# olegroshka/vae-channel-dynamics

Hardware: AMD Instinct MI355X
Metric: images/sec SDXL-VAE train step @256x256 (tracking on) (higher is better)
Workload: dtype f32

## Files before the change

### vae-channel-dynamics_amd/csrc/wgrad3_wino.hip

```cpp
#include "common.h"
#ifndef VAE_ABLATE
#define VAE_ABLATE 0
#endif
#include <algorithm>
#include <type_traits>

namespace {

constexpr int GCI = 32, GCO = 128, GNT = 512;
constexpr int XS = 20;
constexpr int SXF = 4 * GCI * XS;
constexpr int SYF = 2 * GCO * XS;
constexpr int GSTAGE = SXF + SYF;

template <int XF>
__global__ __launch_bounds__(GNT, 1) void wgrad3_wino_kernel(vae_wgrad_args p, int strips, int64_t nunits) {
  __shared__ __attribute__((aligned(16))) float smem[2 * GSTAGE];

  const int tid = threadIdx.x, lane = tid & 63, wave = tid >> 6;
  const int lr = lane & 31, lh = lane >> 5;
  const vae_conv_geom g = p.g;
  const int tilesN = p.N / GCI, ntile = tilesN * (p.M / GCO);
  int tile, split;
  {
    const int L = blockIdx.x, ns = p.nsplit;
    if (ns % 8 == 0) {
      const int j = L >> 3;
      tile = j % ntile;
      split = (j / ntile) * 8 + (L & 7);
    } else if ((ns == 2 || ns == 4) && ntile % (8 / ns) == 0) {
      split = (L & 7) % ns;
      tile = (L >> 3) * (8 / ns) + (L & 7) / ns;
    } else {
      tile = L % ntile;
      split = L / ntile;
    }
  }
  const int tm = tile / tilesN, tn = tile % tilesN;
  const int m0 = tm * GCO, n0 = tn * GCI;
  const int64_t per = (nunits + p.nsplit - 1) / p.nsplit;
  const int64_t ubeg = split * per, uend = min(nunits, ubeg + per);
  const int nu = (int)max((int64_t)0, uend - ubeg);
  const int upi = (g.Ho / 2) * strips;
  const bool do_bias = (p.bias_partial != nullptr) && tn == 0;

  const int xx = tid & 15, xq = (tid >> 4) & 7, xr = tid >> 7;
  const bool xe_role = tid < 128 && (tid & 8) == 0;
  const int ex = 16 + (tid & 1), er = (tid >> 1) & 3;
  const int yq = tid >> 4;
  const auto rsX = VAE_BUF_RSRC(p.X, (size_t)g.B * g.Hs * g.Ws * g.Cs * 4u);
  const auto rsY = VAE_BUF_RSRC(p.dY, (size_t)g.B * g.Ho * g.Wo * p.ldy * 4u);
  struct Stg {
    f32x4 rx, rxe, ry[2];
    int b;
    bool xin, xein;
  };
  const f32x4 z4 = {0.f, 0.f, 0.f, 0.f};
  Stg s0{z4, z4, {z4, z4}, -1, false, false}, s1 = s0;
  f32x4 bsum = z4;
  f32x4 rsc = {1.f, 1.f, 1.f, 1.f}, rsh = z4;
  int sc_b = -1;
  int ub = (int)(ubeg / upi), uty = (int)((ubeg - (int64_t)ub * upi) / strips), ustrip = (int)((ubeg - (int64_t)ub * upi) % strips);
  const unsigned thrX = ((xr * g.Ws + xx) * g.Cs + n0 + 4 * xq) * 4u, thrE = ((er * g.Ws + ex) * g.Cs + n0 + 4 * xq) * 4u;
  const unsigned thrY = (xx * p.ldy + m0 + 4 * yq) * 4u, rowY = (unsigned)g.Wo * p.ldy * 4u;
  const int tfX = (xr == 0 ? 1 : 0) | (xr == 3 ? 2 : 0) | (xx == 0 ? 4 : 0) | 16;
  const int tfE = xe_role ? ((er == 0 ? 1 : 0) | (er == 3 ? 2 : 0) | (ex == 17 ? 8 : 0) | 16) : 31;
  auto load_unit = [&](int k, Stg& r) {
    const bool ok = k < nu;
    const int b = ub, ty = uty, x0 = ustrip * 16;
    if (++ustrip == strips) {
      ustrip = 0;
      if (++uty == g.Ho / 2) {
        uty = 0;
        ++ub;
      }
    }
    r.b = ok ? b : -1;
    const int uf = (ty == 0 ? 1 : 0) | (2 * ty + 2 >= g.Hs ? 2 : 0) | (x0 == 0 ? 4 : 0) | (x0 + 16 >= g.Ws ? 8 : 0) | (ok ? 0 : 16);
    const unsigned baseX = (unsigned)((b * g.Hs + 2 * ty - 1) * g.Ws + x0 - 1) * (unsigned)g.Cs * 4u;
    const unsigned baseY = (unsigned)((b * g.Ho + 2 * ty) * g.Wo + x0) * (unsigned)p.ldy * 4u;
    r.xin = (tfX & uf) == 0;
    r.rx = VAE_BUF_LOAD4(rsX, r.xin ? baseX + thrX : BUF_OOB);
    r.xein = (tfE & uf) == 0;
    r.rxe = VAE_BUF_LOAD4(rsX, r.xein ? baseX + thrE : BUF_OOB);
#pragma unroll
    for (int a = 0; a < 2; ++a) r.ry[a] = VAE_BUF_LOAD4(rsY, ok ? baseY + a * rowY + thrY : BUF_OOB);
  };
  auto xform = [&](f32x4 v, bool in) {
    if (XF != VAE_XF_NONE) {
#pragma unroll
      for (int e = 0; e < 4; ++e) {
        float u = v[e] * rsc[e] + rsh[e];
        if (XF == VAE_XF_AFFINE_SILU) u = silu_f(u);
        v[e] = in ? u : 0.f;
      }
    }
    return v;
  };
  auto store_unit = [&](float* st, const Stg& r) {
    float* sx = st;
    float* sy = st + SXF;
    if (XF != VAE_XF_NONE && r.b >= 0 && r.b != sc_b) {
      sc_b = r.b;
      rsc = *reinterpret_cast<const f32x4*>(p.scale + (int64_t)sc_b * g.Cs + n0 + 4 * xq);
      rsh = *reinterpret_cast<const f32x4*>(p.shift + (int64_t)sc_b * g.Cs + n0 + 4 * xq);
    }
    const f32x4 v = xform(r.rx, r.xin);
#pragma unroll
    for (int e = 0; e < 4; ++e) sx[(xr * GCI + 4 * xq + e) * XS + xx] = v[e];
    if (xe_role) {
      const f32x4 ve = xform(r.rxe, r.xein);
#pragma unroll
      for (int e = 0; e < 4; ++e) sx[(er * GCI + 4 * xq + e) * XS + ex] = ve[e];
    }
#pragma unroll
    for (int a = 0; a < 2; ++a) {
#pragma unroll
      for (int e = 0; e < 4; ++e) sy[(a * GCO + 4 * yq + e) * XS + xx] = r.ry[a][e];
      if (do_bias) bsum += r.ry[a];
    }
  };

  const int wi = wave >> 1, jh = wave & 1;
  const int vr1 = wi == 0 ? 0 : (wi == 2 ? 2 : 1), vr2 = wi == 0 ? 2 : (wi == 1 ? 2 : (wi == 2 ? 1 : 3));
  const int voff1 = (vr1 * GCI + lr) * XS + 8 * lh, voff2 = (vr2 * GCI + lr) * XS + 8 * lh;
  const int dr1 = wi == 3 ? 1 : 0;

  f32x16 acc[2][4];
#pragma unroll
  for (int pi = 0; pi < 2; ++pi)
#pragma unroll
    for (int nb = 0; nb < 4; ++nb)
#pragma unroll
      for (int e = 0; e < 16; ++e) acc[pi][nb][e] = 0.f;

  load_unit(0, s0);
  store_unit(smem, s0);
  load_unit(1, s1);
  __syncthreads();

  auto run = [&](auto WI, auto JH) {
    constexpr int wic = decltype(WI)::value, jhc = decltype(JH)::value;
    constexpr bool two = wic == 1 || wic == 2;
    constexpr bool vplus = wic == 1;
    auto step = [&](int k, const Stg& cur, Stg& nxt) {
      const float* cx = smem + (k & 1) * GSTAGE;
      const float* cy = cx + SXF;
      float* nst = smem + ((k + 1) & 1) * GSTAGE;
      f32x4 rd[2][2];
      auto read_d = [&](int nb, f32x4 (&d)[2][2]) {
        const int doff = (dr1 * GCO + nb * 32 + lr) * XS + 8 * lh;
#pragma unroll
        for (int c = 0; c < 2; ++c) {
          d[0][c] = *reinterpret_cast<const f32x4*>(&cy[doff + 4 * c]);
          if (two) d[1][c] = *reinterpret_cast<const f32x4*>(&cy[doff + GCO * XS + 4 * c]);
        }
      };
      auto build_b = [&](const f32x4 (&d)[2][2], f32x4 (&b4)[2]) {
        float rc[8];
#pragma unroll
        for (int c = 0; c < 2; ++c)
#pragma unroll
          for (int e = 0; e < 4; ++e) rc[4 * c + e] = !two ? d[0][c][e] : (vplus ? d[0][c][e] + d[1][c][e] : d[0][c][e] - d[1][c][e]);
#pragma unroll
        for (int e = 0; e < 4; ++e) {
          if (jhc == 0) {
            b4[0][e] = rc[2 * e];
            b4[1][e] = rc[2 * e] + rc[2 * e + 1];
          } else {
            b4[0][e] = rc[2 * e] - rc[2 * e + 1];
            b4[1][e] = rc[2 * e + 1];
          }
        }
      };
      f32x4 a4[2], bb[2][2];
      {
        f32x4 u1[3], u2[3];
#pragma unroll
        for (int c = 0; c < 3; ++c) {
          u1[c] = *reinterpret_cast<const f32x4*>(&cx[voff1 + 4 * c]);
          u2[c] = *reinterpret_cast<const f32x4*>(&cx[voff2 + 4 * c]);
        }
        float rc[12];
#pragma unroll
        for (int c = 0; c < 3; ++c)
#pragma unroll
          for (int e = 0; e < 4; ++e) rc[4 * c + e] = vplus ? u1[c][e] + u2[c][e] : u1[c][e] - u2[c][e];
        __builtin_amdgcn_sched_barrier(0);
        read_d(0, rd);
#pragma unroll
        for (int e = 0; e < 4; ++e) {
          if (jhc == 0) {
            a4[0][e] = rc[2 * e] - rc[2 * e + 2];
            a4[1][e] = rc[2 * e + 1] + rc[2 * e + 2];
          } else {
            a4[0][e] = rc[2 * e + 2] - rc[2 * e + 1];
            a4[1][e] = rc[2 * e + 1] - rc[2 * e + 3];
          }
        }
        build_b(rd, bb[0]);
        read_d(1, rd);
      }
      if (!(VAE_ABLATE & 2) && wave < 4) store_unit(nst, cur);
#pragma unroll
      for (int nb = 0; nb < 4; ++nb) {
        __builtin_amdgcn_sched_barrier(0);
        if (nb == 1) {
          if (!(VAE_ABLATE & 1)) load_unit(k + 2, nxt);
          __builtin_amdgcn_sched_barrier(0);
        }
        if (nb == 3 && wave >= 4) {
          if (!(VAE_ABLATE & 2)) store_unit(nst, cur);
          __builtin_amdgcn_sched_barrier(0);
        }
        if (nb < 3) build_b(rd, bb[(nb + 1) & 1]);
        if (nb < 2) read_d(nb + 2, rd);
#pragma unroll
        for (int pi = 0; pi < 2; ++pi)
#pragma unroll
          for (int e = 0; e < 4; ++e) acc[pi][nb] = __builtin_amdgcn_mfma_f32_32x32x2f32(a4[pi][e], bb[nb & 1][pi][e], acc[pi][nb], 0, 0, 0);
#pragma unroll
        for (int i = 0; i < 4; ++i) {
          __builtin_amdgcn_sched_group_barrier(0x008, 1, 0);
          __builtin_amdgcn_sched_group_barrier(0x002, 3, 0);
        }
        __builtin_amdgcn_sched_group_barrier(0x100, 4, 0);
        __builtin_amdgcn_sched_group_barrier(0x008, 4, 0);
        __builtin_amdgcn_sched_barrier(0);
      }
      if (!(VAE_ABLATE & 16)) __syncthreads();
    };
    int k = 0;
    for (; k + 1 < nu; k += 2) {
      step(k, s1, s0);
      step(k + 1, s0, s1);
    }
    if (k < nu) step(k, s1, s0);
  };
  {
    using J0 = std::integral_constant<int, 0>;
    using J1 = std::integral_constant<int, 1>;
    switch (wave) {
      case 0: run(std::integral_constant<int, 0>{}, J0{}); break;
      case 1: run(std::integral_constant<int, 0>{}, J1{}); break;
      case 2: run(std::integral_constant<int, 1>{}, J0{}); break;
      case 3: run(std::integral_constant<int, 1>{}, J1{}); break;
      case 4: run(std::integral_constant<int, 2>{}, J0{}); break;
      case 5: run(std::integral_constant<int, 2>{}, J1{}); break;
      case 6: run(std::integral_constant<int, 3>{}, J0{}); break;
      default: run(std::integral_constant<int, 3>{}, J1{}); break;
    }
  }

  float* __restrict__ O = p.partial + (int64_t)split * 16 * p.N * p.M;
#pragma unroll
  for (int pi = 0; pi < 2; ++pi) {
    const int pos = wi * 4 + 2 * jh + pi;
#pragma unroll
    for (int nb = 0; nb < 4; ++nb)
#pragma unroll
      for (int e = 0; e < 16; ++e) {
        const int ci = n0 + (e & 3) + 8 * (e >> 2) + 4 * lh;
        O[((int64_t)pos * p.N + ci) * p.M + m0 + nb * 32 + lr] = acc[pi][nb][e];
      }
  }
  if (do_bias) {
#pragma unroll
    for (int e = 0; e < 4; ++e) {
      float s = bsum[e];
#pragma unroll
      for (int o = 1; o < 16; o <<= 1) s += __shfl_xor(s, o, 64);
      if (xx == 0) p.bias_partial[(int64_t)split * p.M + m0 + 4 * yq + e] = s;
    }
  }
}

}

bool wgrad3_wino_eligible(const vae_wgrad_args& a) {
  const vae_conv_geom& g = a.g;
  if (a.prec != VAE_PREC_F32 || a.X16 != nullptr || a.dY16 != nullptr || a.dY == nullptr || a.batch != 1 || a.alpha != 1.0f) return false;
  if (g.taps != 9 || g.stride != 1 || g.pad_t != 1 || g.pad_l != 1 || g.mode != VAE_MODE_FWD) return false;
  if (a.tapmask != 0 || a.y_step > 1 || g.Ho != g.Hs || g.Wo != g.Ws) return false;
  if (g.Ho % 2 != 0 || g.Wo % 16 != 0 || a.N % GCI != 0 || a.M % GCO != 0 || g.Cs % 4 != 0 || a.ldy % 4 != 0) return false;
  if (!aligned16(a.X) || !aligned16(a.dY)) return false;
  if ((size_t)g.B * g.Hs * g.Ws * g.Cs * 4u >= BUF_MAX || (size_t)g.B * g.Ho * g.Wo * a.ldy * 4u >= BUF_MAX) return false;
  return true;
}

int64_t wgrad3_wino_units(const vae_conv_geom& g) { return (int64_t)g.B * (g.Ho / 2) * (g.Wo / 16); }

int launch_wgrad3_wino(const vae_wgrad_args& a, hipStream_t st) {
  const vae_conv_geom& g = a.g;
  const int64_t nunits = wgrad3_wino_units(g);
  dim3 grid((unsigned)((a.M / GCO) * (a.N / GCI) * a.nsplit), 1, 1);
  const int strips = g.Wo / 16;
  if (a.xf == VAE_XF_NONE) hipLaunchKernelGGL(wgrad3_wino_kernel<VAE_XF_NONE>, grid, dim3(GNT), 0, st, a, strips, nunits);
  else if (a.xf == VAE_XF_AFFINE) hipLaunchKernelGGL(wgrad3_wino_kernel<VAE_XF_AFFINE>, grid, dim3(GNT), 0, st, a, strips, nunits);
  else hipLaunchKernelGGL(wgrad3_wino_kernel<VAE_XF_AFFINE_SILU>, grid, dim3(GNT), 0, st, a, strips, nunits);
  return 0;
}
```

Baseline: 104.4.

## Defer last channel-block MFMAs of waves 4-7 past the barrier into next step

For waves 4-7, which store the next stage late in the step, the MFMAs for the last one or two channel blocks (default two) are held back and issued at the start of the following step, after the __syncthreads. The goal is to shorten those waves' critical path before the barrier so all waves reach the sync sooner, with the deferred matrix work overlapping the next step's LDS reads. The a4/bb operands move out of the step so they persist across steps, and a final flush runs after the loop. Optional timing instrumentation is added but compiled only when VAE_WGRAD_TIMING is defined.

Result: faster. 106.7 (median of 6 runs) (+2.1%).

```diff
diff --git a/vae-channel-dynamics_amd/csrc/wgrad3_wino.hip b/vae-channel-dynamics_amd/csrc/wgrad3_wino.hip
--- a/vae-channel-dynamics_amd/csrc/wgrad3_wino.hip
+++ b/vae-channel-dynamics_amd/csrc/wgrad3_wino.hip
@@ -1,6 +1,9 @@
 #include "common.h"
 #ifndef VAE_ABLATE
 #define VAE_ABLATE 0
+#endif
+#ifndef VAE_WGRAD_DEFER
+#define VAE_WGRAD_DEFER 2
 #endif
 #include <algorithm>
 #include <type_traits>
@@ -43,6 +46,18 @@
   const int nu = (int)max((int64_t)0, uend - ubeg);
   const int upi = (g.Ho / 2) * strips;
   const bool do_bias = (p.bias_partial != nullptr) && tn == 0;
+#ifdef VAE_WGRAD_TIMING
+  constexpr int TS0 = 2, TSN = 8;
+  const bool tw = (tid & 255) == 0 && blockIdx.x < 8 && p.out != nullptr;
+  unsigned long long* const tout = reinterpret_cast<unsigned long long*>(p.out) + (blockIdx.x * 2 + (tid >> 8)) * (4 + TSN * 5);
+  unsigned long long tst[5];
+  const unsigned long long te0 = __builtin_amdgcn_s_memtime(), tr0 = __builtin_amdgcn_s_memrealtime();
+#define GSTAMP(i) do { __builtin_amdgcn_sched_barrier(0); tst[i] = __builtin_amdgcn_s_memtime(); __builtin_amdgcn_sched_barrier(0); } while (0)
+#define GSTAMPS_OUT(k) do { if (tw && (k) >= TS0 && (k) < TS0 + TSN) { _Pragma("unroll") for (int i_ = 0; i_ < 5; ++i_) tout[4 + ((k) - TS0) * 5 + i_] = tst[i_]; } } while (0)
+#else
+#define GSTAMP(i) do { } while (0)
+#define GSTAMPS_OUT(k) do { } while (0)
+#endif
 
   const int xx = tid & 15, xq = (tid >> 4) & 7, xr = tid >> 7;
   const bool xe_role = tid < 128 && (tid & 8) == 0;
@@ -143,10 +158,32 @@
     constexpr int wic = decltype(WI)::value, jhc = decltype(JH)::value;
     constexpr bool two = wic == 1 || wic == 2;
     constexpr bool vplus = wic == 1;
+    constexpr int ndef = wic >= 2 ? VAE_WGRAD_DEFER : 0;
+    static_assert(ndef >= 0 && ndef <= 2, "bb holds the operands of two channel blocks");
+    f32x4 a4[2], bb[2][2];
+    if (ndef > 0) {
+      a4[0] = a4[1] = z4;
+      bb[0][0] = bb[0][1] = bb[1][0] = bb[1][1] = z4;
+    }
+    auto held_back = [&]() {
+#pragma unroll
+      for (int e = 0; e < 4; ++e)
+#pragma unroll
+        for (int nb = 4 - ndef; nb < 4; ++nb)
+#pragma unroll
+          for (int pi = 0; pi < 2; ++pi) acc[pi][nb] = __builtin_amdgcn_mfma_f32_32x32x2f32(a4[pi][e], bb[nb & 1][pi][e], acc[pi][nb], 0, 0, 0);
+    };
     auto step = [&](int k, const Stg& cur, Stg& nxt) {
       const float* cx = smem + (k & 1) * GSTAGE;
       const float* cy = cx + SXF;
       float* nst = smem + ((k + 1) & 1) * GSTAGE;
+      GSTAMP(0);
+      if (ndef > 0) {
+        __builtin_amdgcn_sched_barrier(0);
+        held_back();
+        __builtin_amdgcn_sched_barrier(0);
+      }
+      GSTAMP(1);
       f32x4 rd[2][2];
       auto read_d = [&](int nb, f32x4 (&d)[2][2]) {
         const int doff = (dr1 * GCO + nb * 32 + lr) * XS + 8 * lh;
@@ -173,7 +210,6 @@
           }
         }
       };
-      f32x4 a4[2], bb[2][2];
       {
         f32x4 u1[3], u2[3];
 #pragma unroll
@@ -202,6 +238,7 @@
         read_d(1, rd);
       }
       if (!(VAE_ABLATE & 2) && wave < 4) store_unit(nst, cur);
+      GSTAMP(2);
 #pragma unroll
       for (int nb = 0; nb < 4; ++nb) {
         __builtin_amdgcn_sched_barrier(0);
@@ -215,19 +252,24 @@
         }
         if (nb < 3) build_b(rd, bb[(nb + 1) & 1]);
         if (nb < 2) read_d(nb + 2, rd);
-#pragma unroll
-        for (int pi = 0; pi < 2; ++pi)
-#pragma unroll
-          for (int e = 0; e < 4; ++e) acc[pi][nb] = __builtin_amdgcn_mfma_f32_32x32x2f32(a4[pi][e], bb[nb & 1][pi][e], acc[pi][nb], 0, 0, 0);
-#pragma unroll
-        for (int i = 0; i < 4; ++i) {
-          __builtin_amdgcn_sched_group_barrier(0x008, 1, 0);
-          __builtin_amdgcn_sched_group_barrier(0x002, 3, 0);
-        }
-        __builtin_amdgcn_sched_group_barrier(0x100, 4, 0);
-        __builtin_amdgcn_sched_group_barrier(0x008, 4, 0);
-        __builtin_amdgcn_sched_barrier(0);
-      }
+        if (nb < 4 - ndef) {
+#pragma unroll
+          for (int pi = 0; pi < 2; ++pi)
+#pragma unroll
+            for (int e = 0; e < 4; ++e) acc[pi][nb] = __builtin_amdgcn_mfma_f32_32x32x2f32(a4[pi][e], bb[nb & 1][pi][e], acc[pi][nb], 0, 0, 0);
+#pragma unroll
+          for (int i = 0; i < 4; ++i) {
+            __builtin_amdgcn_sched_group_barrier(0x008, 1, 0);
+            __builtin_amdgcn_sched_group_barrier(0x002, 3, 0);
+          }
+          __builtin_amdgcn_sched_group_barrier(0x100, 4, 0);
+          __builtin_amdgcn_sched_group_barrier(0x008, 4, 0);
+        }
+        __builtin_amdgcn_sched_barrier(0);
+        if (nb == 3 - ndef) GSTAMP(3);
+      }
+      GSTAMP(4);
+      GSTAMPS_OUT(k);
       if (!(VAE_ABLATE & 16)) __syncthreads();
     };
     int k = 0;
@@ -236,6 +278,7 @@
       step(k + 1, s0, s1);
     }
     if (k < nu) step(k, s1, s0);
+    if (ndef > 0 && nu > 0) held_back();
   };
   {
     using J0 = std::integral_constant<int, 0>;
@@ -252,6 +295,14 @@
     }
   }
 
+#ifdef VAE_WGRAD_TIMING
+  if (tw) {
+    tout[0] = te0;
+    tout[1] = __builtin_amdgcn_s_memtime();
+    tout[2] = tr0;
+    tout[3] = __builtin_amdgcn_s_memrealtime();
+  }
+#endif
   float* __restrict__ O = p.partial + (int64_t)split * 16 * p.N * p.M;
 #pragma unroll
   for (int pi = 0; pi < 2; ++pi) {
```
